# eltoto1219/vltk

Hardware: AMD Instinct MI355X
Metric: images/sec FRCNN feature extraction, 800x1333 batch (higher is better)
Workload: dtype f16; 1 GPU; configs[1]: ResNet-101-C4 fp16 (the reference has no FPN: SURVEY.md D1), 32 synthetic 800x1333 images per GPU per step, R=300 RPN proposals through the Res5 head, max 100 detections/img, seeded synthetic weights; global_batch=32, parallelism=image-sharded x1, all-gather of output blocks

## Files before the change

### include/vltk_hip.h

```cpp
#ifndef VLTK_HIP_H
#define VLTK_HIP_H

#include <stddef.h>
#include <stdint.h>

#ifdef __cplusplus
extern "C" {
#endif

#define VK_OK 0
#define VK_EINVAL 1
#define VK_ENOTIMPL 2
#define VK_ENONFINITE 3
#define VK_EWEIGHTS 4
#define VK_EHIP 5
#define VK_ENOMEM 6

typedef enum { VK_F32 = 0, VK_F16 = 1, VK_I64 = 2, VK_I32 = 3, VK_BF16 = 4 } vk_dtype;
typedef enum { VK_ACT_NONE = 0, VK_ACT_RELU = 1, VK_ACT_GELU = 2 , VK_ACT_TANH = 3 } vk_act;

#define VK_MAX_ANCHOR_DIM 8
#define VK_MAX_NMS_THRESH 8

typedef struct vk_config {
// ... 121 lines not shown
                 vk_dtype *dtype, int64_t *shape, int *ndim);

int vk_memcpy_d2d(void *dst_dev, const void *src_dev, size_t bytes, void *stream);

int vk_enable_stage_timing(vk_handle *h, int enable);
int vk_get_stage_timing(vk_handle *h, float *ms6);

#define VK_NUM_KERNEL_BUCKETS 12
int vk_enable_kernel_timing(vk_handle *h, int enable);
int vk_get_kernel_timing(vk_handle *h, int64_t *launches, double *ms, double *flops, double *bytes, int reset);


size_t vk_packed_weight_bytes(int cout, int cin, int kh, int kw, int groups, vk_dtype dt);
int vk_packed_cout(int cout);
int vk_conv_slice_channels(int cin, int groups);
int vk_pack_conv_weight(const float *w_oihw_host, const float *bn_host, const float *bias_host,
                        int cout, int cin, int kh, int kw, int groups, vk_dtype dt,
                        void *w_packed_host, float *bias_packed_host);

int vk_conv2d(const void *x, int N, int H, int W, int cin,
              const void *w_packed, const float *bias_packed, const void *residual,
              void *y, int cout, int ldy, int kh, int kw, int stride, int pad, int dil, int groups,
              int relu, vk_dtype dt, vk_dtype out_dt, void *stream);

#define VK_ROUTE_GENERIC 0
#define VK_ROUTE_RING 1
#define VK_ROUTE_DUO 2
#define VK_ROUTE_WS 3
#define VK_ROUTE_GEMM4 4
#define VK_ROUTE_PANEL 5
#define VK_ROUTE_BLK 6
int vk_conv_route(int N, int H, int W, int cin, int cin2, int has_residual, int fused_mean, int cout, int ldy, int kh, int kw,
                  int stride, int pad, int dil, int groups, int relu, vk_dtype dt, vk_dtype out_dt);

int vk_conv1x1_dual(const void *x1, int cin1, const void *x2, int cin2, long M,
                    const void *w_packed, const float *bias_packed, const void *residual,
                    void *y, int cout, int relu, void *stream);

int vk_bottleneck64(const void *x, int N, int H, int W, int cin, int proj,
                    const void *w1_packed, const float *b1_packed, const void *w2_packed, const float *b2_packed,
                    const void *w3_packed, const float *b3_packed, void *y, void *stream);

int vk_fuse_shortcut(int cin, int cin_shortcut, int cout, int stride, vk_dtype dt);
int vk_bottleneck64_eligible(int cin, int cmid, int cout, int stride, int dil, int groups, int proj, int fused_shortcut,
                             long N, int H, int W, vk_dtype dt);

size_t vk_conv1x1_meanpool_workspace_bytes(int N, int HW, int cout);
int vk_conv1x1_meanpool(const void *x, int N, int HW, int cin, const void *w_packed, const float *bias_packed,
                        const void *residual, int cout, int relu, float *out_mean,
                        void *workspace, size_t workspace_bytes, void *stream);


int vk_linear(const void *x, long M, int K, const void *w_packed, const float *bias_packed, const void *residual,
              void *y, int N, int ldy, int act, vk_dtype dt, vk_dtype out_dt, void *stream);
int vk_layernorm(const void *x, int ldx, const float *gamma, const float *beta, void *y, int ldy, int M, int C,
                 float eps, float scale, int accumulate, vk_dtype dt, void *stream);
int vk_embed_layernorm(const int64_t *input_ids, const int64_t *token_type_ids, int B, int L, const void *word,
                       const void *position, const void *token_type, const float *gamma, const float *beta,
                       void *y, int C, float eps, vk_dtype dt, void *stream);
int vk_attention(const void *q, int ldq, const void *k, int ldk, const void *v, int ldv, const float *mask,
                 void *out, int ldo, int B, int heads, int Lq, int Lk, int d, vk_dtype dt, void *stream);


int vk_roi_align(const void *const *maps, const int32_t *Hs, const int32_t *Ws, const float *scales, int levels,
                 int N, int C, const float *rois, const int32_t *roi_levels, int K, int P, int sampling_ratio,
                 int aligned, void *out, vk_dtype dt, void *stream);
// ... 115 lines not shown
```

### vltk_amd/_lib.py

```python
import ctypes as C
import os

_HERE = os.path.dirname(os.path.abspath(__file__))
LIB_PATH = os.path.join(_HERE, "libvltk_hip.so")
if os.environ.get("VLTK_AMD_LIB"):
    LIB_PATH = os.environ["VLTK_AMD_LIB"]
elif os.environ.get("VLTK_AMD_ABLATION_LIB") == "1":
    LIB_PATH = LIB_PATH.replace("libvltk_hip.so", "libvltk_hip_ablation.so")

VK_OK, VK_EINVAL, VK_ENOTIMPL, VK_ENONFINITE, VK_EWEIGHTS, VK_EHIP, VK_ENOMEM = range(7)
VK_F32, VK_F16, VK_I64, VK_I32, VK_BF16 = 0, 1, 2, 3, 4
VK_ACT_NONE, VK_ACT_RELU, VK_ACT_GELU, VK_ACT_TANH = 0, 1, 2, 3
VK_ROUTE_GENERIC, VK_ROUTE_RING, VK_ROUTE_DUO, VK_ROUTE_WS, VK_ROUTE_GEMM4, VK_ROUTE_PANEL, VK_ROUTE_BLK = range(7)
VK_MAX_ANCHOR_DIM = 8
VK_MAX_NMS_THRESH = 8
VK_MAX_IGNOREY = 64
VK_SELECT_CLASS_MAX, VK_SELECT_PER_CLASS, VK_SELECT_DETECTIONS = 0, 1, 2

_EXC = {
    VK_EINVAL: ValueError,
    VK_ENOTIMPL: NotImplementedError,
    VK_ENONFINITE: AssertionError,
    VK_EWEIGHTS: OSError,
    VK_EHIP: RuntimeError,
# ... 51 lines not shown
    "vk_load_weights": (_I, [_P, C.c_char_p, _P, C.POINTER(C.c_int64), _I, _I]),
    "vk_finalize": (_I, [_P]),
    "vk_destroy": (_I, [_P]),
    "vk_set_option": (_I, [_P, C.c_char_p, _I]),
    "vk_get_option": (_I, [_P, C.c_char_p, C.POINTER(_I)]),
    "vk_option_check": (_I, [C.c_char_p, _I]),
    "vk_option_default": (_I, [C.c_char_p, C.POINTER(_I)]),
    "vk_num_weights": (_I, [_P, C.POINTER(_I)]),
    "vk_weight_name": (_I, [_P, _I, C.POINTER(C.c_char_p)]),
    "vk_forward": (_I, [_P, _P, _I, _I, _I, _P, _P, C.POINTER(vk_roi_params), C.POINTER(vk_outputs), _P]),
    "vk_forward_begin": (_I, [_P, _P, _I, _I, _I, _P, _P, C.POINTER(vk_roi_params), C.POINTER(vk_outputs), _P,
                              C.POINTER(C.c_int64)]),
    "vk_forward_begin_ignorey": (_I, [_P, _P, _I, _I, _I, _P, _P, C.POINTER(vk_roi_params), C.POINTER(vk_outputs), _P,
                                      C.POINTER(C.c_int64), C.POINTER(vk_ignorey)]),
    "vk_forward_begin_select": (_I, [_P, _P, _I, _I, _I, _P, _P, C.POINTER(vk_select_params), C.POINTER(vk_outputs), _P,
                                     C.POINTER(C.c_int64), C.POINTER(vk_ignorey)]),
    "vk_forward_boxes_begin": (_I, [_P, _P, _I, _I, _I, _P, _P, _P, _I, _P, C.POINTER(vk_outputs), _P, C.POINTER(C.c_int64)]),
    "vk_forward_grid_begin": (_I, [_P, _P, _I, _I, _I, _P, _P, _I, _I, C.POINTER(vk_outputs), _P, C.POINTER(C.c_int64)]),
    "vk_grid_pool": (_I, [_P, _I, _I, _I, _I, _I, _P, _P, _I, _I, _I, _P, _I, _P, _P]),
    "vk_forward_end": (_I, [_P, C.c_int64]),
    "vk_given_boxes_ingest": (_I, [_P, _P, _P, _P, _I, _I, _P, _P, _P, _I, _I, _F, _I, _P, _P]),
    "vk_given_box_outputs": (_I, [_P, _P, _P, _P, _P, _P, _P, _P, _I, _I, _I, C.POINTER(vk_outputs), _P]),
    "vk_get_stage": (_I, [_P, C.c_char_p, C.POINTER(_P), C.POINTER(_I), C.POINTER(C.c_int64), C.POINTER(_I)]),
    "vk_memcpy_d2d": (_I, [_P, _P, _SZ, _P]),
    "vk_enable_stage_timing": (_I, [_P, _I]),
    "vk_get_stage_timing": (_I, [_P, C.POINTER(_F)]),
    "vk_enable_kernel_timing": (_I, [_P, _I]),
    "vk_get_kernel_timing": (_I, [_P, C.POINTER(C.c_int64), C.POINTER(_D), C.POINTER(_D), C.POINTER(_D), _I]),
    "vk_packed_weight_bytes": (_SZ, [_I, _I, _I, _I, _I, _I]),
    "vk_conv_slice_channels": (_I, [_I, _I]),
    "vk_packed_cout": (_I, [_I]),
    "vk_pack_conv_weight": (_I, [_P, _P, _P, _I, _I, _I, _I, _I, _I, _P, _P]),
    "vk_conv_route": (_I, [_I] * 18),
    "vk_conv1x1_dual": (_I, [_P, _I, _P, _I, C.c_long, _P, _P, _P, _P, _I, _I, _P]),
    "vk_bottleneck64": (_I, [_P, _I, _I, _I, _I, _I, _P, _P, _P, _P, _P, _P, _P, _P]),
    "vk_fuse_shortcut": (_I, [_I, _I, _I, _I, _I]),
    "vk_bottleneck64_eligible": (_I, [_I, _I, _I, _I, _I, _I, _I, _I, C.c_long, _I, _I, _I]),
    "vk_conv1x1_meanpool_workspace_bytes": (_SZ, [_I, _I, _I]),
    "vk_conv1x1_meanpool": (_I, [_P, _I, _I, _I, _P, _P, _P, _I, _I, _P, _P, _SZ, _P]),
    "vk_linear": (_I, [_P, C.c_long, _I, _P, _P, _P, _P, _I, _I, _I, _I, _I, _P]),
    "vk_layernorm": (_I, [_P, _I, _P, _P, _P, _I, _I, _I, _F, _F, _I, _I, _P]),
    "vk_embed_layernorm": (_I, [_P, _P, _I, _I, _P, _P, _P, _P, _P, _P, _I, _F, _I, _P]),
    "vk_attention": (_I, [_P, _I, _P, _I, _P, _I, _P, _P, _I, _I, _I, _I, _I, _I, _I, _P]),
    "vk_roi_align": (_I, [_P, _P, _P, _P, _I, _I, _I, _P, _P, _I, _I, _I, _I, _P, _I, _P]),
    "vk_assign_levels": (_I, [_P, _I, _I, _I, _I, _F, _I, _P, _P]),
    "vk_upsample2x_add": (_I, [_P, _P, _P, _I, _I, _I, _I, _I, _I, _I, _P]),
    "vk_subsample2": (_I, [_P, _P, _I, _I, _I, _I, _I, _P]),
    "vk_relu_copy": (_I, [_P, _P, C.c_long, _I, _P]),
    "vk_rpn_multilevel_workspace_bytes": (_SZ, [_I, _I, _I, _I]),
    "vk_rpn_proposals_multilevel": (_I, [_P, _P, _P, _P, _I, _I, _P, _P, _I, _P, _P, _F, _P, _P, _F, _D, _I, _I, _P, _P, _P, _P, _P, _SZ, _P]),
    "vk_rpn_proposals_multilevel_ignorey": (_I, [_P, _P, _P, _P, _I, _I, _P, _P, _I, _P, _P, _F, _P, _P, _F, _D, _I, _I, _P, _P, _P, _P,
                                                 _P, _SZ, _P, C.POINTER(vk_ignorey)]),
    "vk_conv2d": (_I, [_P, _I, _I, _I, _I, _P, _P, _P, _P, _I, _I, _I, _I, _I, _I, _I, _I, _I, _I, _I, _P]),
    "vk_nchw_to_nhwc": (_I, [_P, _I, _I, _I, _I, _P, _I, _P]),
    "vk_nhwc_to_nchw": (_I, [_P, _I, _I, _I, _I, _P, _I, _P]),
    "vk_packed_stem_bytes": (_SZ, [_I, _I]),
    "vk_pack_stem_weight": (_I, [_P, _P, _I, _I, _P, _P]),
    "vk_stem": (_I, [_P, _I, _I, _I, _P, _P, _I, _I, _P, _I, _P, _SZ, _P]),
    "vk_stem_workspace_bytes": (_SZ, [_I, _I, _I, _I, _I]),
    "vk_stem_out_hw": (None, [_I, _I, _I, C.POINTER(_I), C.POINTER(_I)]),
    "vk_preprocess": (_I, [_P, _P, _P, _I, _I, _I, C.POINTER(_F), C.POINTER(_F), _F, _P, _P]),
    "vk_maxpool3x3s2": (_I, [_P, _I, _I, _I, _I, _I, _P, _I, _P]),
    "vk_rpn_workspace_bytes": (_SZ, [_I, _I, _I]),
    "vk_rpn_proposals": (_I, [_P, _I, _P, _I, _I, _I, _I, _I, _P, _I, _F, _P, C.POINTER(_F), _F, _D, _I, _I,
                              _P, _P, _P, _P, _P, _SZ, _P]),
    "vk_rpn_proposals_ignorey": (_I, [_P, _I, _P, _I, _I, _I, _I, _I, _P, _I, _F, _P, C.POINTER(_F), _F, _D, _I, _I,
# ... 54 lines not shown
```

### vltk_amd/csrc/conv3x3_panel.hip

```cpp
#include <cstdio>
#include <type_traits>
#include <vector>

#include "vk_common.h"

namespace vk {

typedef _Float16 half8 __attribute__((ext_vector_type(8)));
typedef float floatx4 __attribute__((ext_vector_type(4)));
typedef _Float16 half4 __attribute__((ext_vector_type(4)));
typedef unsigned uintx4 __attribute__((ext_vector_type(4)));

struct PanelK {
    const char *x;
    const char *w;
    const float *bias;
    const char *res;
    char *y;
    int H, W, HW, M;
    int cin_bytes, ldy;
    int dil;
    int cstages;
    int wrow_bytes;
    int relu;
    int m_tiles, n_tiles;
    unsigned long *stamps;
    unsigned *tile_ctr;
    int static_tiles;
    unsigned ctr_last;
};

constexpr int P_NW = 6;
constexpr int P_WSLOT = 256 * 64;

#define VKP_GLDS16(gptr, lptr)                                                                         \
    __builtin_amdgcn_global_load_lds((const __attribute__((address_space(1))) void *)(gptr),          \
                                     (__attribute__((address_space(3))) void *)(lptr), 16, 0, 0)

template <int J, int PP>
constexpr int panel_in_window() {
    int c = 0;
    for (int d = 1; d <= P_NW - 2; ++d) {
        int t = ((J - d) % 9 + 9) % 9;
        if (t < PP) ++c;
    }
    return c;
}
template <int J>
constexpr int last_w_in_window() {
    int c = 0;
    for (int d = 1; d <= P_NW - 2; ++d) {
        int t = J - d;
        if (t < 0 || t + P_NW < 9) ++c;
    }
    return 2 * c;
}

template <int N>
__device__ __forceinline__ void vm_wait() {
    static_assert(N >= 0 && N <= 15, "vmcnt immediate");
    asm volatile("s_waitcnt vmcnt(%0)" ::"n"(N) : "memory");
}

template <int PP, int DBG, int TAG = 0, int MI = 8>
__global__ __launch_bounds__(512, 2) void conv3x3_panel_kernel(PanelK p) {
    extern __shared__ __attribute__((aligned(16))) char smem[];
    static_assert(MI == 8 || MI == 9, "8 or 9 row tiles per wave");
    static_assert(MI == 8 || !(DBG & 8), "the LDS-staged epilogue is written for 128-row halves");
    constexpr int TILE = 2 * MI * 16;
    constexpr int PROWS = PP * 128;
    constexpr int HALO = (PROWS - TILE) / 2;
    constexpr int PBYTES = PROWS * 64;
    constexpr int WBASE = 2 * PBYTES;
    constexpr bool ZROW = PP == 3;
    constexpr int ZOFF = WBASE + P_NW * P_WSLOT;

    int bid = blockIdx.x;
    const int nwg = p.m_tiles * p.n_tiles;
    unsigned long st_k0 = 0;
    if constexpr (DBG & 4) asm volatile("s_memrealtime %0\n\ts_waitcnt lgkmcnt(0)" : "=s"(st_k0)::"memory");
    if constexpr (PP == 3) {
        if (p.tile_ctr && bid >= p.static_tiles) {
            int *mail = reinterpret_cast<int *>(smem + 2 * PP * 128 * 64 + P_NW * P_WSLOT + 128);
            if (threadIdx.x == 0) {
                const unsigned v = atomicAdd(p.tile_ctr, 1u);
                if (v == p.ctr_last) *p.tile_ctr = 0u;
                *mail = p.static_tiles + (int)v;
            }
            __syncthreads();
            bid = __builtin_amdgcn_readfirstlane(*mail);
            if (bid >= nwg) return;
        }
    }
    const int q = nwg >> 3, r = nwg & 7, xcd = bid & 7;
    const int t_ = (xcd < r ? xcd * (q + 1) : r * (q + 1) + (xcd - r) * q) + (bid >> 3);
    const int n_tile = t_ % p.n_tiles, m_tile = t_ / p.n_tiles;
    const int m0 = m_tile * TILE, n0 = n_tile * 256;

    const int tid = threadIdx.x, lane = tid & 63;
    const int wave = __builtin_amdgcn_readfirstlane(tid >> 6);
    const int wr = wave >> 2, wc = wave & 3;
    const int g = lane >> 4, j = lane & 15;

    unsigned vm0 = 0, vm1 = 0, vm2 = 0;

    const int lrow = lane >> 2;
    const int lchunk = (lane & 3) ^ ((-(lrow >> 2)) & 3);
    const int pm_first = m0 - HALO + wave * 16 + lrow;
    const unsigned wsrc0 = (unsigned)(n0 + wave * 32 + lrow) * (unsigned)p.wrow_bytes + lchunk * 16;
    const unsigned wstep = 16u * p.wrow_bytes;
    auto req_panel = [&](int cs, int piece) {
        int pf = pm_first;
        asm volatile("" : "+v"(pf));
        const int m = min(max(pf + piece * 128, 0), p.M - 1);
        const unsigned off = (unsigned)m * (unsigned)p.cin_bytes + cs * 64 + lchunk * 16;
        VKP_GLDS16(p.x + off, smem + (cs & 1) * PBYTES + (piece * 8 + wave) * 1024);
    };
    auto req_w = [&](int slot, int cs, int tap, int i) {
        const unsigned koff = (unsigned)(tap * p.cstages + cs) * 64;
        unsigned wb_ = wsrc0;
        asm volatile("" : "+v"(wb_));
        VKP_GLDS16(p.w + (wb_ + i * wstep + koff), smem + WBASE + slot * P_WSLOT + (wave * 2 + i) * 1024);
    };

    const unsigned lds0 = (unsigned)(unsigned long)(__attribute__((address_space(3))) char *)smem;
    [[maybe_unused]] const unsigned zrow = lds0 + ZOFF;
    if constexpr (ZROW) {
        if (tid < 16) *reinterpret_cast<unsigned *>(smem + ZOFF + tid * 4) = 0u;
        asm volatile("s_waitcnt lgkmcnt(0)" ::: "memory");
    }
    unsigned w_a[2];
#pragma unroll
    for (int par = 0; par < 2; ++par) {
        const int wrow = wc * 64 + (j >> 2) * 8 + par * 4 + (j & 3);
        w_a[par] = lds0 + WBASE + wrow * 64 + ((g ^ ((-(wrow >> 2)) & 3)) << 4);
    }
    const int jbase = HALO + wr * (MI * 16) + j;
    auto x_addr_of = [&](int parity, int tap) -> unsigned {
        const int shift = ((tap / 3 - 1) * p.W + (tap % 3 - 1)) * p.dil;
        int jb = jbase;
        asm volatile("" : "+v"(jb));
        const int rb = jb + shift;
        return lds0 + parity * PBYTES + (rb << 6) + ((g ^ ((-(rb >> 2)) & 3)) << 4);
    };

    floatx4 acc[MI][4];
#pragma unroll
    for (int mi = 0; mi < MI; ++mi)
#pragma unroll
        for (int ni = 0; ni < 4; ++ni) acc[mi][ni] = floatx4{0.f, 0.f, 0.f, 0.f};
    half8 wa[4], wb[4], xw[MI == 9 ? 5 : 4];
    const int CS = p.cstages;

#define VKP_DSR(dst, addr, OFF) asm volatile("ds_read_b128 %0, %1 offset:" #OFF : "=v"(dst) : "v"(addr))
#define VKP_DSRX(dst, addr, OFF, TW, J_, MI_)                                                        \
    do {                                                                                             \
        if constexpr (ZROW && !(DBG & 1)) {                                                          \
            unsigned m_, ad_;                                                                        \
            const unsigned zc_ = zrow - (OFF);                                                       \
            asm volatile("v_bfe_i32 %0, %1, %2, 1" : "=v"(m_) : "v"(TW), "n"(((J_) % 3) * 9 + (MI_))); \
            asm volatile("v_bfi_b32 %0, %1, %2, %3" : "=v"(ad_) : "v"(m_), "v"(addr), "s"(zc_));    \
            VKP_DSR(dst, ad_, OFF);                                                                  \
        } else                                                                                       \
            VKP_DSR(dst, addr, OFF);                                                                 \
    } while (0)
#define VKP_WAIT3(reg) asm volatile("s_waitcnt lgkmcnt(3)" : "+v"(reg))
#define VKP_WAIT4(reg) asm volatile("s_waitcnt lgkmcnt(4)" : "+v"(reg))
#define VKP_SB() __builtin_amdgcn_sched_barrier(0)
#define VKP_MMA_ROW(MI, XR, WF, TM)                                                                  \
    do {                                                                                             \
        if constexpr (!(DBG & 1) && !ZROW) {                                                         \
            uintx4 u_ = __builtin_bit_cast(uintx4, XR);                                              \
            const bool v_ = ((TM) >> (MI)) & 1u;                                                     \
            u_[0] = v_ ? u_[0] : 0u;                                                                 \
            u_[1] = v_ ? u_[1] : 0u;                                                                 \
            u_[2] = v_ ? u_[2] : 0u;                                                                 \
            u_[3] = v_ ? u_[3] : 0u;                                                                 \
            XR = __builtin_bit_cast(half8, u_);                                                      \
        }                                                                                            \
        __builtin_amdgcn_s_setprio(1);                                                               \
        _Pragma("unroll") for (int ni = 0; ni < 4; ++ni) acc[MI][ni] =                               \
            __builtin_amdgcn_mfma_f32_16x16x32_f16(WF[ni], XR, acc[MI][ni], 0, 0, 0);                \
        __builtin_amdgcn_s_setprio(0);                                                               \
    } while (0)
#define VKP_READ_W(WF, so)                              \
    do {                                                \
        unsigned a0_ = w_a[0], a1_ = w_a[1];            \
        asm volatile("" : "+v"(a0_), "+v"(a1_));        \
        a0_ += so;                                      \
        a1_ += so;                                      \
        VKP_DSR(WF[0], a0_, 0);                         \
        VKP_DSR(WF[1], a1_, 0);                         \
        VKP_DSR(WF[2], a0_, 2048);                      \
        VKP_DSR(WF[3], a1_, 2048);                      \
    } while (0)

    auto tap_mask = [&](auto j_c) -> unsigned {
        constexpr int J = decltype(j_c)::value;
        unsigned tw = J < 3 ? vm0 : (J < 6 ? vm1 : vm2);
        asm volatile("" : "+v"(tw));
        return tw >> ((J % 3) * 9);
    };
    auto tap_word = [&](auto j_c) -> unsigned {
        constexpr int J = decltype(j_c)::value;
        unsigned tw = J < 3 ? vm0 : (J < 6 ? vm1 : vm2);
        asm volatile("" : "+v"(tw));
        return tw;
    };
    auto pre = [&](auto last_c, auto odd_c, auto j_c, unsigned xa, unsigned &xa_next, const half8 (&wcur)[4]) {
        constexpr bool LAST = decltype(last_c)::value;
        constexpr int ODD = decltype(odd_c)::value;
        constexpr int J = decltype(j_c)::value;
        const unsigned tm = ZROW ? 0u : tap_mask(j_c);
        [[maybe_unused]] const unsigned tw = ZROW ? tap_word(j_c) : 0u;
        constexpr bool has_next = !(LAST && J == 8);
        if constexpr (has_next) xa_next = (J == 8) ? x_addr_of(1 - ODD, 0) : x_addr_of(ODD, J + 1);
        VKP_DSRX(xw[3], xa, 3072, tw, J, 3); VKP_WAIT3(xw[0]); VKP_SB(); VKP_MMA_ROW(0, xw[0], wcur, tm); VKP_SB();
        VKP_DSRX(xw[0], xa, 4096, tw, J, 4); VKP_WAIT3(xw[1]); VKP_SB(); VKP_MMA_ROW(1, xw[1], wcur, tm); VKP_SB();
        VKP_DSRX(xw[1], xa, 5120, tw, J, 5); VKP_WAIT3(xw[2]); VKP_SB(); VKP_MMA_ROW(2, xw[2], wcur, tm); VKP_SB();
        VKP_DSRX(xw[2], xa, 6144, tw, J, 6); VKP_WAIT3(xw[3]); VKP_SB(); VKP_MMA_ROW(3, xw[3], wcur, tm); VKP_SB();
        if constexpr (MI == 9) {
            VKP_DSRX(xw[3], xa, 7168, tw, J, 7); VKP_DSRX(xw[4], xa, 8192, tw, J, 8); VKP_WAIT4(xw[0]); VKP_SB(); VKP_MMA_ROW(4, xw[0], wcur, tm); VKP_SB();
            asm volatile("s_waitcnt lgkmcnt(0)" : "+v"(xw[1]), "+v"(xw[2]), "+v"(xw[3]), "+v"(xw[MI == 9 ? 4 : 3])::"memory");
        } else {
            VKP_DSRX(xw[3], xa, 7168, tw, J, 7); VKP_WAIT3(xw[0]); VKP_SB(); VKP_MMA_ROW(4, xw[0], wcur, tm); VKP_SB();
            asm volatile("s_waitcnt lgkmcnt(0)" : "+v"(xw[1]), "+v"(xw[2]), "+v"(xw[3])::"memory");
        }
        VKP_SB();
        if constexpr (has_next) {
            constexpr int OUT = LAST ? last_w_in_window<J>() : 2 * (P_NW - 2) + panel_in_window<J, PP>();
            vm_wait<OUT>();
            if constexpr (!(DBG & 48) || ((DBG & 16) && J % 3 == 2)) asm volatile("s_barrier" ::: "memory");
        }
// ... 23 lines not shown
        VKP_MMA_ROW(6, xw[2], wcur, tm);
        VKP_SB();
        if constexpr (issue_w) req_w(SLOT, cs + (J + P_NW) / 9, (J + P_NW) % 9, 1);
        VKP_DSRX(xw[2], xa_next, 2048, twn, JN, 2);
        VKP_SB();
        VKP_MMA_ROW(7, xw[3], wcur, tm);
        VKP_SB();
        if constexpr (MI == 9) {
            VKP_MMA_ROW(8, xw[MI == 9 ? 4 : 3], wcur, tm);
            VKP_SB();
        }
    };
    auto wset = [&](auto u_c) -> half8(&)[4] {
        if constexpr (decltype(u_c)::value % 2 == 0)
            return wa;
        else
            return wb;
    };
#define VKP_IC(V) std::integral_constant<int, (V)> {}
#define VKP_UNIT(LP, LC, U)                                                                                          \
    post(LP, VKP_IC(((U) - 1) / 9), VKP_IC(((U) - 1) % 9), cs + ((U) - 1) / 9, xan, wset(VKP_IC((U) - 1)), wset(VKP_IC(U)));  \
    xa = xan;                                                                                                        \
    pre(LC, VKP_IC((U) / 9), VKP_IC((U) % 9), xa, xan, wset(VKP_IC(U)));
    using T_ = std::integral_constant<bool, true>;
    using F_ = std::integral_constant<bool, false>;

#pragma unroll
    for (int q2 = 0; q2 < PP; ++q2) req_panel(0, q2);
#pragma unroll
    for (int st = 0; st < P_NW; ++st) {
        req_w(st, 0, st, 0);
        req_w(st, 0, st, 1);
    }
    if (p.HW >= MI * 16 + p.W) {
        const int mbase = m0 + wr * (MI * 16);
        const int rem0 = mbase % p.HW, ho0 = rem0 / p.W, wo0 = rem0 - ho0 * p.W;
        const float rcpw = 1.0f / (float)p.W;
#pragma unroll
        for (int mi = 0; mi < MI; ++mi) {
            const int xcol = wo0 + mi * 16 + j;
            int q = (int)((float)xcol * rcpw), wo = xcol - q * p.W;
            if (wo >= p.W) {
                wo -= p.W;
                ++q;
            }
            if (wo < 0) {
                wo += p.W;
                --q;
            }
            int ho = ho0 + q;
            if (ho >= p.H) ho -= p.H;
            const unsigned c0 = (unsigned)(wo - p.dil) < (unsigned)p.W, c1 = 1u, c2 = (unsigned)(wo + p.dil) < (unsigned)p.W;
            const unsigned cw = mbase + mi * 16 + j < p.M ? (c0 << mi) | (c1 << (9 + mi)) | (c2 << (18 + mi)) : 0u;
            vm0 |= (unsigned)(ho - p.dil) < (unsigned)p.H ? cw : 0u;
            vm1 |= cw;
            vm2 |= (unsigned)(ho + p.dil) < (unsigned)p.H ? cw : 0u;
        }
    } else {
#pragma unroll
        for (int mi = 0; mi < MI; ++mi) {
            const int m = m0 + wr * (MI * 16) + mi * 16 + j;
            if (m < p.M) {
                const int n_img = m / p.HW;
                const int rem = m - n_img * p.HW;
                const int ho = rem / p.W, wo = rem - ho * p.W;
#pragma unroll
                for (int tap = 0; tap < 9; ++tap) {
// ... 27 lines not shown
    for (; cs + 2 < CS; cs += 2) {
        VKP_UNIT(F_{}, F_{}, 1) VKP_UNIT(F_{}, F_{}, 2) VKP_UNIT(F_{}, F_{}, 3) VKP_UNIT(F_{}, F_{}, 4) VKP_UNIT(F_{}, F_{}, 5)
        VKP_UNIT(F_{}, F_{}, 6) VKP_UNIT(F_{}, F_{}, 7) VKP_UNIT(F_{}, F_{}, 8) VKP_UNIT(F_{}, F_{}, 9) VKP_UNIT(F_{}, F_{}, 10)
        VKP_UNIT(F_{}, F_{}, 11) VKP_UNIT(F_{}, F_{}, 12) VKP_UNIT(F_{}, F_{}, 13) VKP_UNIT(F_{}, F_{}, 14) VKP_UNIT(F_{}, F_{}, 15)
        VKP_UNIT(F_{}, F_{}, 16) VKP_UNIT(F_{}, F_{}, 17)
        post(F_{}, VKP_IC(1), VKP_IC(8), cs + 1, xan, wb, wa);
        xa = xan;
        pre(F_{}, VKP_IC(0), VKP_IC(0), xa, xan, wa);
    }
    VKP_UNIT(F_{}, F_{}, 1) VKP_UNIT(F_{}, F_{}, 2) VKP_UNIT(F_{}, F_{}, 3) VKP_UNIT(F_{}, F_{}, 4) VKP_UNIT(F_{}, F_{}, 5)
    VKP_UNIT(F_{}, F_{}, 6) VKP_UNIT(F_{}, F_{}, 7) VKP_UNIT(F_{}, F_{}, 8) VKP_UNIT(F_{}, T_{}, 9) VKP_UNIT(T_{}, T_{}, 10)
    VKP_UNIT(T_{}, T_{}, 11) VKP_UNIT(T_{}, T_{}, 12) VKP_UNIT(T_{}, T_{}, 13) VKP_UNIT(T_{}, T_{}, 14) VKP_UNIT(T_{}, T_{}, 15)
    VKP_UNIT(T_{}, T_{}, 16) VKP_UNIT(T_{}, T_{}, 17)
    {
        const unsigned tm = ZROW ? 0u : tap_mask(VKP_IC(8));
        VKP_MMA_ROW(5, xw[1], wb, tm);
        VKP_MMA_ROW(6, xw[2], wb, tm);
        VKP_MMA_ROW(7, xw[3], wb, tm);
        if constexpr (MI == 9) VKP_MMA_ROW(8, xw[MI == 9 ? 4 : 3], wb, tm);
    }
    unsigned long st_c1 = 0, st_r1 = 0;
    if constexpr (DBG & 4) asm volatile("s_memtime %0\n\ts_memrealtime %1\n\ts_waitcnt lgkmcnt(0)" : "=s"(st_c1), "=s"(st_r1)::"memory");
#undef VKP_UNIT
#undef VKP_IC
#undef VKP_DSR
#undef VKP_DSRX
#undef VKP_WAIT3
#undef VKP_WAIT4
#undef VKP_MMA_ROW
#undef VKP_READ_W
#undef VKP_SB

    if constexpr (!(DBG & 8)) {
        auto epilogue = [&](auto res_c, auto relu_c, auto full_c) {
            constexpr bool RES = decltype(res_c)::value, RELU = decltype(relu_c)::value, FULL = decltype(full_c)::value;
            const int ch0 = n0 + wc * 64 + g * 8;
            floatx4 bq[2][2];
#pragma unroll
            for (int qn = 0; qn < 2; ++qn) {
                bq[qn][0] = *reinterpret_cast<const floatx4 *>(p.bias + ch0 + qn * 32);
                bq[qn][1] = *reinterpret_cast<const floatx4 *>(p.bias + ch0 + qn * 32 + 4);
            }
#pragma unroll
            for (int mi = 0; mi < MI; ++mi) {
                const long m = m0 + wr * (MI * 16) + mi * 16 + j;
                half8 rr[2];
                if constexpr (RES) {
                    const long mr = min(m, (long)p.M - 1);
#pragma unroll
                    for (int qn = 0; qn < 2; ++qn) rr[qn] = *reinterpret_cast<const half8 *>(p.res + (mr * p.ldy + ch0 + qn * 32) * 2);
                }
#pragma unroll
                for (int qn = 0; qn < 2; ++qn) {
                    floatx4 x0 = acc[mi][2 * qn] + bq[qn][0], x1 = acc[mi][2 * qn + 1] + bq[qn][1];
                    if constexpr (RES) {
                        x0 += __builtin_convertvector(__builtin_shufflevector(rr[qn], rr[qn], 0, 1, 2, 3), floatx4);
                        x1 += __builtin_convertvector(__builtin_shufflevector(rr[qn], rr[qn], 4, 5, 6, 7), floatx4);
                    }
                    half4 h0 = __builtin_convertvector(x0, half4), h1 = __builtin_convertvector(x1, half4);
                    half8 o = __builtin_shufflevector(h0, h1, 0, 1, 2, 3, 4, 5, 6, 7);
                    if constexpr (RELU) o = __builtin_elementwise_max(o, half8{0, 0, 0, 0, 0, 0, 0, 0});
                    if (FULL || m < p.M) *reinterpret_cast<half8 *>(p.y + (m * p.ldy + ch0 + qn * 32) * 2) = o;
                }
            }
        };
        const bool full = m0 + TILE <= p.M;
        auto by_full = [&](auto r_, auto l_) {
            if (full)
                epilogue(r_, l_, std::true_type{});
            else
                epilogue(r_, l_, std::false_type{});
        };
        auto by_relu = [&](auto r_) {
            if (p.relu)
                by_full(r_, std::true_type{});
            else
                by_full(r_, std::false_type{});
        };
        if (p.res)
            by_relu(std::true_type{});
        else
            by_relu(std::false_type{});
    } else {
    asm volatile("s_barrier" ::: "memory");
    floatx4 *stg = reinterpret_cast<floatx4 *>(smem);
    auto load_res = [&](int h, half8 (&rr)[8]) {
#pragma unroll
        for (int i = 0; i < 8; ++i) {
            const int it = tid + 512 * i, row = it >> 5, k8 = it & 31;
            const int m = min(m0 + h * 128 + row, p.M - 1);
            if (p.res)
                rr[i] = *reinterpret_cast<const half8 *>(p.res + ((long)m * p.ldy + n0 + k8 * 8) * 2);
            else
                rr[i] = half8{0, 0, 0, 0, 0, 0, 0, 0};
        }
// ... 63 lines not shown
        }
    }
}

static int panel_pp(const ConvArgs &a, int mi = 8) {
    const int reach = a.dil * (a.W + 1);
    if (mi == 9) return reach <= 48 ? 3 : (reach <= 112 ? 4 : 0);
    return reach <= 64 ? 3 : (reach <= 128 ? 4 : 0);
}

static int panel_mi(const ConvArgs &a, long M, int n_cu) {
    if (panel_pp(a, 9) == 0) return 8;
    if (const char *v = getenv("VK_PANEL_MI")) {
        if (v[0] == '8') return 8;
        if (v[0] == '9') return 9;
    }
    const long nt = a.Cout / 256;
    const long n8 = ((M + 255) / 256 * nt + n_cu - 1) / n_cu, n9 = ((M + 287) / 288 * nt + n_cu - 1) / n_cu;
    if (n8 > 4) return 9;
    return n9 * 9 < n8 * 8 ? 9 : 8;
}

bool conv3x3_panel_eligible(const ConvArgs &a) {
    const char *v = getenv("VK_CONV3X3_PANEL");
    if (v && v[0] == '0') return false;
    if (a.stem || a.dt != VK_F16 || a.out_dt != VK_F16 || a.relu > 1) return false;
    if (a.kh != 3 || a.kw != 3 || a.stride != 1 || a.pad != a.dil) return false;
    if (a.Cout % 256 != 0 || a.ldy != a.Cout || a.Cin % 64 != 0 || a.Cin < 128) return false;
    if (panel_pp(a) == 0) return false;
    if ((long)a.N * a.H * a.W * a.Cin * 2 >= (1L << 32)) return false;
    return true;
}

int launch_conv3x3_panel(const ConvArgs &a, hipStream_t stream) {
    DeviceState *ds = nullptr;
    VK_TRY(device_state(&ds));
    PanelK k;
    k.x = (const char *)a.x;
    k.w = (const char *)a.w;
    k.bias = a.bias;
    k.res = (const char *)a.res;
    k.y = (char *)a.y;
    k.H = a.H;
    k.W = a.W;
    k.HW = a.H * a.W;
    const long M = (long)a.N * a.H * a.W;
    VK_REQUIRE(M > 0 && M < (1L << 31) - 512, VK_EINVAL, "conv3x3_panel: M=%ld out of range", M);
    VK_REQUIRE(M * a.Cin * 2 < (1L << 32) && (long)a.Cout * 9 * a.Cin * 2 < (1L << 32), VK_EINVAL,
               "conv3x3_panel: tensor beyond the 32-bit DMA offsets (M=%ld Cin=%d Cout=%d)", M, a.Cin, a.Cout);
    k.M = (int)M;
    k.cin_bytes = a.Cin * 2;
    k.ldy = a.ldy;
    k.dil = a.dil;
    k.cstages = a.Cin / 32;
    k.wrow_bytes = 9 * a.Cin * 2;
    k.relu = a.relu;
    const int mi = panel_mi(a, M, ds->n_cu), pp = panel_pp(a, mi);
    k.m_tiles = ceil_div(k.M, mi * 32);
    k.n_tiles = a.Cout / 256;
    Timed t;
    VK_TRY(t.begin(stream));
    const int total_tiles = k.m_tiles * k.n_tiles;
    k.tile_ctr = nullptr;
    k.static_tiles = total_tiles;
    int n_wgs = total_tiles;
    const char *dyn_env = getenv("VK_PANEL_DYNAMIC");
    const bool dyn_off = dyn_env && dyn_env[0] == '0';
    if (!dyn_off && pp == 3 && total_tiles >= 16 * 256) {
        VK_TRY(acquire_tile_counter(&k.tile_ctr));
        k.static_tiles = total_tiles * 15 / 16 / 8 * 8;
        n_wgs = total_tiles + (total_tiles / 32 + 63) / 64 * 64;
        k.ctr_last = (unsigned)(n_wgs - k.static_tiles - 1);
    }
    const dim3 grid(n_wgs), block(512);
#ifdef VK_ABLATION
    const int dbg = getenv("VK_CONV256_DBG") ? atoi(getenv("VK_CONV256_DBG")) : 0;
#endif
    const int smem = 2 * pp * 128 * 64 + P_NW * P_WSLOT + (pp == 3 ? 256 : 0);
    k.stamps = nullptr;
#define VKP_LAUNCH(PP_, DBG_, TAG_, MI_)                                                                                                   \
    do {                                                                                                                                   \
        VK_TRY(set_max_lds(conv3x3_panel_kernel<PP_, DBG_, TAG_, MI_>, 2 * PP_ * 128 * 64 + P_NW * P_WSLOT + (PP_ == 3 ? 256 : 0)));        \
        hipLaunchKernelGGL((conv3x3_panel_kernel<PP_, DBG_, TAG_, MI_>), grid, block, smem, stream, k);                                     \
    } while (0)
#ifdef VK_ABLATION
    if (const char *sf = getenv("VK_PANEL_STAMPS"); sf && pp == 3) {
        const size_t nb = (size_t)grid.x * 6 * sizeof(unsigned long);
        VK_CHECK_HIP(hipMalloc((void **)&k.stamps, nb));
        VK_CHECK_HIP(hipMemset(k.stamps, 0, nb));
        if (mi == 9)
            VKP_LAUNCH(3, 4, 0, 9);
        else
            VKP_LAUNCH(3, 4, 0, 8);
        VK_CHECK_HIP(hipStreamSynchronize(stream));
        std::vector<unsigned long> h((size_t)grid.x * 6);
        VK_CHECK_HIP(hipMemcpy(h.data(), k.stamps, nb, hipMemcpyDeviceToHost));
        VK_CHECK_HIP(hipFree(k.stamps));
        if (FILE *f = fopen(sf, "a")) {
            fprintf(f, "# wg k_loop_cycles k_loop_ticks workgroup_ticks ticks_before_k_loop start_tick end_tick (tick = 10 ns)\n");
            for (unsigned w = 0; w < grid.x; ++w)
                fprintf(f, "%u %lu %lu %lu %lu %lu %lu\n", w, h[(size_t)w * 6], h[(size_t)w * 6 + 1], h[(size_t)w * 6 + 2], h[(size_t)w * 6 + 3], h[(size_t)w * 6 + 4],
                        h[(size_t)w * 6 + 5]);
            fclose(f);
        }
    } else if (mi == 8 && pp == 3 && dbg == 8)
        VKP_LAUNCH(3, 8, 0, 8);
    else if (mi == 8 && pp == 3 && dbg == 1)
        VKP_LAUNCH(3, 1, 0, 8);
    else if (mi == 9 && pp == 3 && dbg == 1)
        VKP_LAUNCH(3, 1, 0, 9);
    else if (mi == 9 && pp == 3 && dbg == 16)
        VKP_LAUNCH(3, 16, 0, 9);
    else if (mi == 9 && pp == 3 && dbg == 32)
        VKP_LAUNCH(3, 32, 0, 9);
    else
#endif
    if (mi == 8 && pp == 3 && a.concurrent)
        VKP_LAUNCH(3, 0, 1, 8);
    else if (mi == 8 && pp == 3)
        VKP_LAUNCH(3, 0, 0, 8);
    else if (mi == 8 && a.concurrent)
        VKP_LAUNCH(4, 0, 1, 8);
    else if (mi == 8)
        VKP_LAUNCH(4, 0, 0, 8);
    else if (pp == 3 && a.concurrent)
        VKP_LAUNCH(3, 0, 1, 9);
    else if (pp == 3)
        VKP_LAUNCH(3, 0, 0, 9);
    else if (a.concurrent)
        VKP_LAUNCH(4, 0, 1, 9);
    else
        VKP_LAUNCH(4, 0, 0, 9);
#undef VKP_LAUNCH
    VK_CHECK_HIP(hipGetLastError());
    return t.end(stream, a.concurrent ? 6 : 4, 2.0 * (double)k.M * a.Cout * 9 * a.Cin, k.M, a.Cout, a.Cin, 9, 1,
                 2.0 * ((double)k.M * a.Cin + (double)k.M * a.Cout * (a.res ? 2 : 1) + (double)a.Cout * 9 * a.Cin));
}

}
```

### vltk_amd/csrc/model.hip

```cpp
#include <cmath>
#include <cstdlib>
#include <map>
#include <mutex>
#include <set>
#include <string>
#include <vector>

#include "vk_common.h"

namespace vk {

thread_local KernelTimer *g_timer = nullptr;

hipEvent_t KernelTimer::get() {
    if (pool.empty()) {
        hipEvent_t e = nullptr;
        (void)hipEventCreate(&e);
        all.push_back(e);
        return e;
    }
    hipEvent_t e = pool.back();
    pool.pop_back();
    return e;
}
// ... 714 lines not shown
              const void *residual, void *y, int cout, int ldy, int kh, int kw, int stride, int pad, int dil, int groups,
              int relu, vk_dtype dt, vk_dtype out_dt, void *stream) {
    VK_REQUIRE(kh == kw && kh >= 1 && stride >= 1 && dil >= 1 && pad >= 0 && groups >= 1, VK_EINVAL, "conv2d: bad geometry");
    ConvArgs a;
    fill_conv_args(a, N, H, W, cin, cout, ldy, kh, stride, pad, dil, groups, relu, dt, out_dt);
    VK_REQUIRE(a.Ho > 0 && a.Wo > 0 && N > 0, VK_EINVAL, "conv2d: empty output");
    a.x = x;
    a.w = w_packed;
    a.bias = bias_packed;
    a.res = residual;
    a.y = y;
    return launch_conv(a, (hipStream_t)stream);
}

int vk_conv_route(int N, int H, int W, int cin, int cin2, int has_residual, int fused_mean, int cout, int ldy, int kh, int kw,
                  int stride, int pad, int dil, int groups, int relu, vk_dtype dt, vk_dtype out_dt) {
    if (!(kh == kw && kh >= 1 && stride >= 1 && dil >= 1 && pad >= 0 && groups >= 1 && cin2 >= 0)) {
        set_error("conv_route: bad geometry");
        return -VK_EINVAL;
    }
    static const char here = 0;
    ConvArgs a;
    fill_conv_args(a, N, H, W, cin, cout, ldy, kh, stride, pad, dil, groups, relu, dt, out_dt);
    if (!(a.Ho > 0 && a.Wo > 0 && N > 0)) {
        set_error("conv_route: empty output");
        return -VK_EINVAL;
    }
    a.x = a.w = &here;
    a.res = has_residual ? &here : nullptr;
    a.x2 = cin2 > 0 ? &here : nullptr;
    a.Cin2 = cin2;
    a.pool_part = fused_mean ? (float *)&here : nullptr;
    return conv_route_checked(a);
}

int vk_conv1x1_dual(const void *x1, int cin1, const void *x2, int cin2, long M, const void *w_packed, const float *bias_packed,
                    const void *residual, void *y, int cout, int relu, void *stream) {
    VK_REQUIRE(x1 && x2 && M > 0 && M < (1L << 31), VK_EINVAL, "conv1x1_dual: bad arguments");
    ConvArgs a;
    fill_conv_args(a, 1, 1, (int)M, cin1, cout, cout, 1, 1, 0, 1, 1, relu, VK_F16, VK_F16);
    a.x = x1;
    a.x2 = x2;
    a.Cin2 = cin2;
    a.w = w_packed;
    a.bias = bias_packed;
    a.res = residual;
    a.y = y;
    return launch_conv(a, (hipStream_t)stream);
}

int vk_conv1x1_rows(const void *x1, int cin1, const void *x2, int cin2, long M, const int32_t *m_dev, const int32_t *x2_idx,
                    const void *w_packed, const float *bias_packed, void *y, int cout, int relu, void *stream) {
    VK_REQUIRE(x1 && w_packed && bias_packed && y && M > 0 && M < (1L << 31), VK_EINVAL, "conv1x1_rows: bad arguments");
    VK_REQUIRE(!x2_idx || x2, VK_EINVAL, "conv1x1_rows: a row index needs a second input");
    ConvArgs a;
    fill_conv_args(a, 1, 1, (int)M, cin1, cout, cout, 1, 1, 0, 1, 1, relu, VK_F16, VK_F16);
    a.x = x1;
    a.x2 = x2;
    a.Cin2 = x2 ? cin2 : 0;
    a.w = w_packed;
    a.bias = bias_packed;
    a.y = y;
    VK_REQUIRE(conv_route(a) == VK_ROUTE_GEMM4, VK_EINVAL, "conv1x1_rows: the layer does not run as VK_ROUTE_GEMM4 at %ld rows", M);
    a.m_dev = m_dev;
    a.x2_idx = x2_idx;
    return launch_conv_gemm4(a, (hipStream_t)stream);
// ... 1501 lines not shown
```

### vltk_amd/csrc/vk_common.h

```cpp
#pragma once
#include <hip/hip_runtime.h>

#include <atomic>
#include <cstdarg>
#include <cstdint>
#include <cstdio>
#include <cstring>
#include <vector>

#include "vltk_hip.h"

namespace vk {

void set_error(const char *fmt, ...);

#define VK_CHECK_HIP(expr)                                                                    \
    do {                                                                                      \
        hipError_t _e = (expr);                                                               \
        if (_e != hipSuccess) {                                                               \
            vk::set_error("%s:%d: %s -> %s", __FILE__, __LINE__, #expr, hipGetErrorString(_e)); \
            return VK_EHIP;                                                                   \
        }                                                                                     \
    } while (0)

// ... 28 lines not shown
static inline size_t align_up(size_t v, size_t a) { return (v + a - 1) / a * a; }

constexpr int CONV_BM = 128;
constexpr int CONV_KTILE_BYTES = 128;
constexpr int CONV_COUT_ALIGN = 128;

struct ConvArgs {
    const void *x;
    const void *w;
    const float *bias;
    const void *res;
    void *y;
    int N, H, W, Cin;
    int Ho, Wo, Cout, ldy;
    int kh, kw, stride, pad, dil;
    int groups;
    int concurrent;
    float *pool_part;
    const void *x2;
    int Cin2;
    int relu;
    int stem;
    const int32_t *m_dev;
    const int32_t *x2_idx;
    vk_dtype dt, out_dt;
};
int launch_conv(const ConvArgs &a, hipStream_t stream);
int conv_route(const ConvArgs &a);
int conv_route_checked(const ConvArgs &a);
bool conv256_eligible(const ConvArgs &a);
int launch_conv256(const ConvArgs &a, hipStream_t stream);
bool conv3x3_panel_eligible(const ConvArgs &a);
int launch_conv3x3_panel(const ConvArgs &a, hipStream_t stream);
bool conv_gemm4_eligible(const ConvArgs &a);
int launch_conv_gemm4(const ConvArgs &a, hipStream_t stream);
int acquire_tile_counter(unsigned **ctr);
bool conv256_dual_ok(const ConvArgs &a);
bool conv_duo_eligible(const ConvArgs &a);
int launch_conv_duo(const ConvArgs &a, hipStream_t stream);
bool conv_ws_eligible(const ConvArgs &a);
int launch_conv_ws(const ConvArgs &a, hipStream_t stream);
bool conv3x3_blk_eligible(const ConvArgs &a);
int launch_conv3x3_blk(const ConvArgs &a, hipStream_t stream);
bool bneck_fused_eligible(int cin, int cmid, int cout, int stride, int groups, bool proj, long N, int H, int W, vk_dtype dt);
int launch_bneck_fused(const void *x, int N, int H, int W, int cin, bool proj, const void *w1, const float *b1, const void *w2,
                       const float *b2, const void *w3, const float *b3, void *y, bool concurrent, hipStream_t stream);
bool conv_duo_dual_ok(const ConvArgs &a);
bool conv_duo_pool_ok(const ConvArgs &a);
size_t conv_duo_pool_part_bytes(long M, int Cout);
bool conv_pool_sums_f64(long N, int HW, int Cin, int Cout, bool dual);
bool conv_ws_pool_ok(const ConvArgs &a);
int launch_pool_finish(const float *part, int N, int HoWo, int Cin, int Cout, bool dual, float *out, hipStream_t stream);

struct KernelTimer {
    struct Rec {
        int bucket;
        double flops;
        hipEvent_t e0, e1;
        int M, cout, cin, k, stride;
        double bytes;
    };
    std::vector<Rec> recs;
    std::vector<hipEvent_t> pool;
    std::vector<hipEvent_t> all;
    int64_t launches[VK_NUM_KERNEL_BUCKETS] = {};
    double ms[VK_NUM_KERNEL_BUCKETS] = {};
// ... 165 lines not shown
```

Baseline: 503.9 images/sec.

## Add phase-decomposed panel path for dilation-2 3x3 convs on small maps

Adds a PHASE variant of the 3x3 panel conv kernel for dilation-2 convolutions on small even-sized maps (W<=14), such as the Res5 head on ROI features. Rows are regrouped into four stride-2 parity phases across 16-image groups, so a dilated 3x3 becomes a dense 3x3 on each half-resolution phase. This shrinks the halo to 128 rows and lets tap masks stay in scalar registers. The epilogue scatters outputs back to the original row order, and the MMA path drops the zero-row skip in favour of mask-gated MFMAs with raised priority. Any leftover images that don't fill a group of 16 go through the old kernel. The cost is more index arithmetic and a scattered output write.

```diff
diff --git a/include/vltk_hip.h b/include/vltk_hip.h
--- a/include/vltk_hip.h
+++ b/include/vltk_hip.h
@@ -177,6 +177,7 @@
 #define VK_ROUTE_BLK 6
 int vk_conv_route(int N, int H, int W, int cin, int cin2, int has_residual, int fused_mean, int cout, int ldy, int kh, int kw,
                   int stride, int pad, int dil, int groups, int relu, vk_dtype dt, vk_dtype out_dt);
+int vk_panel_phase_images(int N, int H, int W, int dil);
 
 int vk_conv1x1_dual(const void *x1, int cin1, const void *x2, int cin2, long M,
                     const void *w_packed, const float *bias_packed, const void *residual,
diff --git a/vltk_amd/_lib.py b/vltk_amd/_lib.py
--- a/vltk_amd/_lib.py
+++ b/vltk_amd/_lib.py
@@ -107,6 +107,7 @@
     "vk_packed_cout": (_I, [_I]),
     "vk_pack_conv_weight": (_I, [_P, _P, _P, _I, _I, _I, _I, _I, _I, _P, _P]),
     "vk_conv_route": (_I, [_I] * 18),
+    "vk_panel_phase_images": (_I, [_I, _I, _I, _I]),
     "vk_conv1x1_dual": (_I, [_P, _I, _P, _I, C.c_long, _P, _P, _P, _P, _I, _I, _P]),
     "vk_bottleneck64": (_I, [_P, _I, _I, _I, _I, _I, _P, _P, _P, _P, _P, _P, _P, _P]),
     "vk_fuse_shortcut": (_I, [_I, _I, _I, _I, _I]),
diff --git a/vltk_amd/csrc/conv3x3_panel.hip b/vltk_amd/csrc/conv3x3_panel.hip
--- a/vltk_amd/csrc/conv3x3_panel.hip
+++ b/vltk_amd/csrc/conv3x3_panel.hip
@@ -28,7 +28,20 @@
     unsigned *tile_ctr;
     int static_tiles;
     unsigned ctr_last;
+    int groups;
+    unsigned rcp_w2;
 };
+
+struct PhaseBlk {
+    int qy, qx, row;
+};
+__device__ __forceinline__ PhaseBlk phase_blk(const PanelK &p, int gb) {
+    const int W2 = p.W >> 1, Q = p.HW >> 2;
+    const int ph = (gb >= Q ? 1 : 0) + (gb >= 2 * Q ? 1 : 0) + (gb >= 3 * Q ? 1 : 0);
+    const int q = gb - ph * Q;
+    const int qy = (int)(((unsigned)q * p.rcp_w2) >> 16), qx = q - qy * W2;
+    return {qy, qx, (2 * qy + (ph >> 1)) * p.W + 2 * qx + (ph & 1)};
+}
 
 constexpr int P_NW = 6;
 constexpr int P_WSLOT = 256 * 64;
@@ -62,10 +75,11 @@
     asm volatile("s_waitcnt vmcnt(%0)" ::"n"(N) : "memory");
 }
 
-template <int PP, int DBG, int TAG = 0, int MI = 8>
+template <int PP, int DBG, int TAG = 0, int MI = 8, int PHASE = 0>
 __global__ __launch_bounds__(512, 2) void conv3x3_panel_kernel(PanelK p) {
     extern __shared__ __attribute__((aligned(16))) char smem[];
     static_assert(MI == 8 || MI == 9, "8 or 9 row tiles per wave");
+    static_assert(!PHASE || (PP == 4 && MI == 8 && !(DBG & 9)), "the phase form: halo 128 = (W / 2 + 1) * 16 at W = 14, 256-row tiles");
     static_assert(MI == 8 || !(DBG & 8), "the LDS-staged epilogue is written for 128-row halves");
     constexpr int TILE = 2 * MI * 16;
     constexpr int PROWS = PP * 128;
@@ -79,9 +93,9 @@
     const int nwg = p.m_tiles * p.n_tiles;
     unsigned long st_k0 = 0;
     if constexpr (DBG & 4) asm volatile("s_memrealtime %0\n\ts_waitcnt lgkmcnt(0)" : "=s"(st_k0)::"memory");
-    if constexpr (PP == 3) {
+    if constexpr (PP == 3 || PHASE) {
         if (p.tile_ctr && bid >= p.static_tiles) {
-            int *mail = reinterpret_cast<int *>(smem + 2 * PP * 128 * 64 + P_NW * P_WSLOT + 128);
+            int *mail = reinterpret_cast<int *>(smem + (PHASE ? 0 : 2 * PP * 128 * 64 + P_NW * P_WSLOT + 128));
             if (threadIdx.x == 0) {
                 const unsigned v = atomicAdd(p.tile_ctr, 1u);
                 if (v == p.ctr_last) *p.tile_ctr = 0u;
@@ -89,6 +103,7 @@
             }
             __syncthreads();
             bid = __builtin_amdgcn_readfirstlane(*mail);
+            if constexpr (PHASE) __syncthreads();
             if (bid >= nwg) return;
         }
     }
@@ -109,7 +124,43 @@
     const int pm_first = m0 - HALO + wave * 16 + lrow;
     const unsigned wsrc0 = (unsigned)(n0 + wave * 32 + lrow) * (unsigned)p.wrow_bytes + lchunk * 16;
     const unsigned wstep = 16u * p.wrow_bytes;
+    int g0 = 0, gb0 = 0;
+    if constexpr (PHASE) {
+        g0 = (m0 >> 4) / p.HW;
+        gb0 = (m0 >> 4) - g0 * p.HW;
+    }
+    auto blk_of = [&](int off, int &G) -> int {
+        int t = gb0 + off;
+        G = g0;
+        while (t < 0) {
+            t += p.HW;
+            --G;
+        }
+        while (t >= p.HW) {
+            t -= p.HW;
+            ++G;
+        }
+        if (G < 0) G = 0, t = 0;
+        if (G >= p.groups) G = p.groups - 1, t = p.HW - 1;
+        return t;
+    };
+    [[maybe_unused]] unsigned ps_lane = 0, ps_blk[PP] = {};
+    if constexpr (PHASE) {
+        ps_lane = (unsigned)(lrow * p.HW) * (unsigned)p.cin_bytes + lchunk * 16;
+#pragma unroll
+        for (int q2 = 0; q2 < PP; ++q2) {
+            int G;
+            const int t = blk_of(wave - HALO / 16 + q2 * 8, G);
+            ps_blk[q2] = __builtin_amdgcn_readfirstlane((unsigned)(G * 16 * p.HW + phase_blk(p, t).row) * (unsigned)p.cin_bytes);
+        }
+    }
     auto req_panel = [&](int cs, int piece) {
+        if constexpr (PHASE) {
+            unsigned pl = ps_lane;
+            asm volatile("" : "+v"(pl));
+            VKP_GLDS16(p.x + (pl + (ps_blk[piece] + cs * 64)), smem + (cs & 1) * PBYTES + (piece * 8 + wave) * 1024);
+            return;
+        }
         int pf = pm_first;
         asm volatile("" : "+v"(pf));
         const int m = min(max(pf + piece * 128, 0), p.M - 1);
@@ -137,7 +188,7 @@
     }
     const int jbase = HALO + wr * (MI * 16) + j;
     auto x_addr_of = [&](int parity, int tap) -> unsigned {
-        const int shift = ((tap / 3 - 1) * p.W + (tap % 3 - 1)) * p.dil;
+        const int shift = PHASE ? ((tap / 3 - 1) * (p.W >> 1) + (tap % 3 - 1)) * 16 : ((tap / 3 - 1) * p.W + (tap % 3 - 1)) * p.dil;
         int jb = jbase;
         asm volatile("" : "+v"(jb));
         const int rb = jb + shift;
@@ -169,6 +220,15 @@
 #define VKP_SB() __builtin_amdgcn_sched_barrier(0)
 #define VKP_MMA_ROW(MI, XR, WF, TM)                                                                  \
     do {                                                                                             \
+        if constexpr (PHASE == 2) {                                                                  \
+            if (((TM) >> (MI)) & 1u) {                           \
+                __builtin_amdgcn_s_setprio(1);                                                       \
+                _Pragma("unroll") for (int ni = 0; ni < 4; ++ni) acc[MI][ni] =                       \
+                    __builtin_amdgcn_mfma_f32_16x16x32_f16(WF[ni], XR, acc[MI][ni], 0, 0, 0);        \
+                __builtin_amdgcn_s_setprio(0);                                                       \
+            }                                                                                        \
+            break;                                                                                   \
+        }                                                                                            \
         if constexpr (!(DBG & 1) && !ZROW) {                                                         \
             uintx4 u_ = __builtin_bit_cast(uintx4, XR);                                              \
             const bool v_ = ((TM) >> (MI)) & 1u;                                                     \
@@ -198,7 +258,10 @@
     auto tap_mask = [&](auto j_c) -> unsigned {
         constexpr int J = decltype(j_c)::value;
         unsigned tw = J < 3 ? vm0 : (J < 6 ? vm1 : vm2);
-        asm volatile("" : "+v"(tw));
+        if constexpr (PHASE)
+            asm volatile("" : "+s"(tw));
+        else
+            asm volatile("" : "+v"(tw));
         return tw >> ((J % 3) * 9);
     };
     auto tap_word = [&](auto j_c) -> unsigned {
@@ -288,7 +351,22 @@
         req_w(st, 0, st, 0);
         req_w(st, 0, st, 1);
     }
-    if (p.HW >= MI * 16 + p.W) {
+    if constexpr (PHASE) {
+        unsigned u0 = 0, u1 = 0, u2 = 0;
+#pragma unroll
+        for (int mi = 0; mi < MI; ++mi) {
+            int G;
+            const PhaseBlk b = phase_blk(p, blk_of(wr * MI + mi, G));
+            const unsigned c0 = b.qx >= 1, c2 = b.qx + 1 < (p.W >> 1);
+            const unsigned cw = m0 + (wr * MI + mi) * 16 < p.M ? (c0 << mi) | (1u << (9 + mi)) | (c2 << (18 + mi)) : 0u;
+            u0 |= b.qy >= 1 ? cw : 0u;
+            u1 |= cw;
+            u2 |= b.qy + 1 < (p.H >> 1) ? cw : 0u;
+        }
+        vm0 = __builtin_amdgcn_readfirstlane(u0);
+        vm1 = __builtin_amdgcn_readfirstlane(u1);
+        vm2 = __builtin_amdgcn_readfirstlane(u2);
+    } else if (p.HW >= MI * 16 + p.W) {
         const int mbase = m0 + wr * (MI * 16);
         const int rem0 = mbase % p.HW, ho0 = rem0 / p.W, wo0 = rem0 - ho0 * p.W;
         const float rcpw = 1.0f / (float)p.W;
@@ -382,6 +460,7 @@
 #undef VKP_SB
 
     if constexpr (!(DBG & 8)) {
+        if constexpr (PHASE) asm volatile("" : "+s"(g0), "+s"(gb0));
         auto epilogue = [&](auto res_c, auto relu_c, auto full_c) {
             constexpr bool RES = decltype(res_c)::value, RELU = decltype(relu_c)::value, FULL = decltype(full_c)::value;
             const int ch0 = n0 + wc * 64 + g * 8;
@@ -394,9 +473,15 @@
 #pragma unroll
             for (int mi = 0; mi < MI; ++mi) {
                 const long m = m0 + wr * (MI * 16) + mi * 16 + j;
+                long mo = m;
+                if constexpr (PHASE) {
+                    int G;
+                    const int t = blk_of(wr * MI + mi, G);
+                    mo = (long)(G * 16 + j) * p.HW + phase_blk(p, t).row;
+                }
                 half8 rr[2];
                 if constexpr (RES) {
-                    const long mr = min(m, (long)p.M - 1);
+                    const long mr = min(mo, (long)p.M - 1);
 #pragma unroll
                     for (int qn = 0; qn < 2; ++qn) rr[qn] = *reinterpret_cast<const half8 *>(p.res + (mr * p.ldy + ch0 + qn * 32) * 2);
                 }
@@ -410,7 +495,7 @@
                     half4 h0 = __builtin_convertvector(x0, half4), h1 = __builtin_convertvector(x1, half4);
                     half8 o = __builtin_shufflevector(h0, h1, 0, 1, 2, 3, 4, 5, 6, 7);
                     if constexpr (RELU) o = __builtin_elementwise_max(o, half8{0, 0, 0, 0, 0, 0, 0, 0});
-                    if (FULL || m < p.M) *reinterpret_cast<half8 *>(p.y + (m * p.ldy + ch0 + qn * 32) * 2) = o;
+                    if (FULL || m < p.M) *reinterpret_cast<half8 *>(p.y + (mo * p.ldy + ch0 + qn * 32) * 2) = o;
                 }
             }
         };
@@ -540,7 +625,31 @@
     return true;
 }
 
+int conv3x3_panel_phase_images(const ConvArgs &a) {
+    const char *v = getenv("VK_PANEL_PHASE");
+    if (v && v[0] == '0') return 0;
+    if (a.dil != 2 || a.H % 2 != 0 || a.W % 2 != 0 || a.W > 14 || a.H > 1024 || a.N < 16) return 0;
+    return a.N / 16 * 16;
+}
+
+static int launch_panel_one(const ConvArgs &a, hipStream_t stream, bool phase);
+
 int launch_conv3x3_panel(const ConvArgs &a, hipStream_t stream) {
+    const int np = conv3x3_panel_phase_images(a);
+    if (np == 0) return launch_panel_one(a, stream, false);
+    ConvArgs b = a;
+    b.N = np;
+    VK_TRY(launch_panel_one(b, stream, true));
+    if (np == a.N) return VK_OK;
+    const size_t rows = (size_t)np * a.H * a.W;
+    b.N = a.N - np;
+    b.x = (const char *)a.x + rows * a.Cin * 2;
+    b.y = (char *)a.y + rows * a.ldy * 2;
+    if (a.res) b.res = (const char *)a.res + rows * a.ldy * 2;
+    return launch_panel_one(b, stream, false);
+}
+
+static int launch_panel_one(const ConvArgs &a, hipStream_t stream, bool phase) {
     DeviceState *ds = nullptr;
     VK_TRY(device_state(&ds));
     PanelK k;
@@ -563,7 +672,9 @@
     k.cstages = a.Cin / 32;
     k.wrow_bytes = 9 * a.Cin * 2;
     k.relu = a.relu;
-    const int mi = panel_mi(a, M, ds->n_cu), pp = panel_pp(a, mi);
+    const int mi = phase ? 8 : panel_mi(a, M, ds->n_cu), pp = phase ? 4 : panel_pp(a, mi);
+    k.groups = phase ? a.N / 16 : 0;
+    k.rcp_w2 = phase ? 65536u / (unsigned)(a.W / 2) + 1u : 0u;
     k.m_tiles = ceil_div(k.M, mi * 32);
     k.n_tiles = a.Cout / 256;
     Timed t;
@@ -574,7 +685,7 @@
     int n_wgs = total_tiles;
     const char *dyn_env = getenv("VK_PANEL_DYNAMIC");
     const bool dyn_off = dyn_env && dyn_env[0] == '0';
-    if (!dyn_off && pp == 3 && total_tiles >= 16 * 256) {
+    if (!dyn_off && (pp == 3 || phase) && total_tiles >= 16 * 256) {
         VK_TRY(acquire_tile_counter(&k.tile_ctr));
         k.static_tiles = total_tiles * 15 / 16 / 8 * 8;
         n_wgs = total_tiles + (total_tiles / 32 + 63) / 64 * 64;
@@ -623,7 +734,16 @@
         VKP_LAUNCH(3, 32, 0, 9);
     else
 #endif
-    if (mi == 8 && pp == 3 && a.concurrent)
+#ifdef VK_ABLATION
+    if (const char *pv = getenv("VK_PANEL_PHASE"); phase && pv && pv[0] == 'A') {
+        VK_TRY(set_max_lds(conv3x3_panel_kernel<4, 0, 0, 8, 1>, smem));
+        hipLaunchKernelGGL((conv3x3_panel_kernel<4, 0, 0, 8, 1>), grid, block, smem, stream, k);
+    } else
+#endif
+    if (phase) {
+        VK_TRY(set_max_lds(conv3x3_panel_kernel<4, 0, 0, 8, 2>, smem));
+        hipLaunchKernelGGL((conv3x3_panel_kernel<4, 0, 0, 8, 2>), grid, block, smem, stream, k);
+    } else if (mi == 8 && pp == 3 && a.concurrent)
         VKP_LAUNCH(3, 0, 1, 8);
     else if (mi == 8 && pp == 3)
         VKP_LAUNCH(3, 0, 0, 8);
diff --git a/vltk_amd/csrc/model.hip b/vltk_amd/csrc/model.hip
--- a/vltk_amd/csrc/model.hip
+++ b/vltk_amd/csrc/model.hip
@@ -770,6 +770,12 @@
     a.Cin2 = cin2;
     a.pool_part = fused_mean ? (float *)&here : nullptr;
     return conv_route_checked(a);
+}
+
+int vk_panel_phase_images(int N, int H, int W, int dil) {
+    ConvArgs a;
+    fill_conv_args(a, N, H, W, 128, 256, 256, 3, 1, dil, dil, 1, 0, VK_F16, VK_F16);
+    return conv3x3_panel_phase_images(a);
 }
 
 int vk_conv1x1_dual(const void *x1, int cin1, const void *x2, int cin2, long M, const void *w_packed, const float *bias_packed,
diff --git a/vltk_amd/csrc/vk_common.h b/vltk_amd/csrc/vk_common.h
--- a/vltk_amd/csrc/vk_common.h
+++ b/vltk_amd/csrc/vk_common.h
@@ -84,6 +84,7 @@
 int launch_conv256(const ConvArgs &a, hipStream_t stream);
 bool conv3x3_panel_eligible(const ConvArgs &a);
 int launch_conv3x3_panel(const ConvArgs &a, hipStream_t stream);
+int conv3x3_panel_phase_images(const ConvArgs &a);
 bool conv_gemm4_eligible(const ConvArgs &a);
 int launch_conv_gemm4(const ConvArgs &a, hipStream_t stream);
 int acquire_tile_counter(unsigned **ctr);
```

Result: faster. 511.9 images/sec (median of 6 runs) (+1.6%).
